# johannah/drqv2

Hardware: AMD Instinct MI355X
Metric: agent updates/sec (batch=256, 9x84x84 obs) (higher is better)
Workload: dtype f32; 1 GPU; cheetah_run batch_size=256/GPU (256 global) 9x84x84 u8 obs, A=6, feature_dim=50, hidden_dim=1024, fp32, use_tb=True; parallelism=dp1, global_batch=256

## Files before the change

drqv2_amd/_lib.py:

```python
import ctypes as C
import os

import torch

HERE = os.path.dirname(os.path.abspath(__file__))
LIB_PATH = os.path.join(HERE, "libdrqv2_hip.so")

c_float_p = C.c_void_p
c_u8_p = C.c_void_p
stream_t = C.c_void_p


class DrqStep(C.Structure):
    _fields_ = [
        ("B", C.c_int), ("global_B", C.c_int), ("C", C.c_int), ("A", C.c_int), ("F", C.c_int), ("H", C.c_int),
        ("obs", c_u8_p), ("next_obs", c_u8_p),
        ("action", c_float_p), ("reward", c_float_p), ("discount", c_float_p),
        ("shift_obs", c_float_p), ("shift_next", c_float_p),
        ("noise_critic", c_float_p), ("noise_actor", c_float_p),
        ("base_grid", c_float_p),
        ("params", c_float_p), ("grads", c_float_p), ("adam_m", c_float_p), ("adam_v", c_float_p),
        ("ws", c_float_p), ("ws_bytes", C.c_size_t),
        ("sums", c_float_p),
        ("lr", C.c_double), ("tau", C.c_double),
# ... 15 lines not shown

PROTOTYPES = {
    "drq_abi_version": (I, []),
    "drq_aug_fwd": (I, [P, P, P, P, I, I, I, I, I, P]),
    "drq_aug_fwd_f32": (I, [P, P, P, P, I, I, I, I, P]),
    "drq_conv1_aug_fwd": (I, [P, P, P, P, P, P, P, P, P, I, I, P]),
    "drq_conv1_aug_fwd_bf16": (I, [P, P, P, P, P, P, P, P, P, I, I, P]),
    "drq_conv1_aug_fwd_bf16_nhwc": (I, [P, P, P, P, P, P, P, P, P, I, I, P]),
    "drq_conv1_aug_fwd_indexed": (I, [P, P, P, P, P, P, P, P, P, P, P, I, I, P]),
    "drq_conv1_aug_fwd_frames": (I, [P, P, L, L, P, P, P, P, P, P, P, P, P, I, I, P]),
    "drq_conv1_aug_fwd_frames_bf16": (I, [P, P, L, L, P, P, P, P, P, P, P, P, P, I, I, P]),
    "drq_conv3x3_fwd": (I, [P, P, P, P, I, I, I, I, I, L, L, L, L, P]),
    "drq_conv3x3_dgrad": (I, [P, P, P, P, I, I, L, L, L, L, P]),
    "drq_conv3x3_fwd_wino": (I, [P, P, P, P, I, I, I, L, L, L, L, P]),
    "drq_conv3x3_dgrad_wino": (I, [P, P, P, P, I, I, L, L, L, L, P]),
    "drq_conv3x3_wgrad_wino": (I, [P, P, P, P, I, I, L, L, L, L, P, SZ, P]),
    "drq_conv3x3_wgrad": (I, [P, P, P, P, I, I, I, I, L, L, L, L, P, SZ, P]),
    "drq_conv3x3_wgrad_ws_bytes": (SZ, []),
    "drq_conv3x3_fwd_bf16": (I, [P, P, P, P, I, I, I, L, L, L, L, P]),
    "drq_conv3x3_dgrad_bf16": (I, [P, P, P, P, I, I, L, L, L, L, P]),
    "drq_conv3x3_wgrad_bf16": (I, [P, P, P, P, I, I, L, L, L, L, P, SZ, P]),
    "drq_conv3x3_fwd_bf16_nhwc": (I, [P, P, P, P, I, I, I, I, I, P]),
    "drq_conv3x3_dgrad_bf16_nhwc": (I, [P, P, P, P, I, I, I, I, L, L, L, L, P]),
    "drq_conv3x3_wgrad_bf16_nhwc": (I, [P, P, P, P, I, I, I, L, L, L, L, P, SZ, P]),
    "drq_gemm_f32": (I, [P, L, I, P, L, I, P, L, I, I, I, I, L, L, L, P, L, I, P, I, L, I, I, I, P, SZ, P]),
    "drq_gemm_batched_f32": (I, [I, P, L, I, P, L, I, P, L, I, I, I, P, I, P, I, P, I, I, I, P, SZ, P]),
    "drq_gemm_batched_bf16": (I, [I, P, L, I, P, L, I, P, L, I, I, I, P, I, P, I, P, I, I, P, SZ, P]),
    "drq_gemm_batched_partial": (I, [I, P, L, I, P, L, I, P, L, I, I, I, P, P, SZ, C.POINTER(I), P]),
    "drq_mlp_fwd": (I, [I, P, L, P, L, P, L, I, I, I, P, I, P, P, C.POINTER(I), P]),
    "drq_mlp_dgrad": (I, [I, P, L, P, L, P, L, I, I, I, P, I, P]),
# ... 49 lines not shown
    "drq_vec_video_record": (I, [P, P, I, P, I, P, I, I, I, L, P]),
    "drq_vec_export_rows": (I, [P, P, P, P, L, L, I, L, I, P, I, P, P, P, P, P]),
    "drq_vec_fill": (I, [P, P, P, P, P, L, L, I, L, L, I, P, P, P, P, P, P]),
    "drq_nstep_gather_frames": (I, [P, P, L, P, P, P, P, I, I, L, I, F, P, P, P, P, P, P]),
    "drq_relu_mask_pad": (I, [P, P, P, L, I, I, P]),
    "drq_conv1_dgrad": (I, [P, P, P, I, P]),
    "drq_aug_bwd_f32": (I, [P, P, P, P, I, I, I, I, P]),
    "drq_tanh_bwd": (I, [P, P, P, L, P]),
    "drq_dormant_scores": (I, [P, L, I, I, P, P]),
    "drq_dormant_count": (I, [P, I, F, P, P, P]),
    "drq_lerp_flat": (I, [P, P, L, F, P]),
    "drq_param_layout": (I, [I, I, I, I, C.POINTER(L), I]),
    "drq_step_ws_bytes": (SZ, [I, I, I, I, I]),
    "drq_step_ws_offset": (L, [I, I, I, I, I, I]),
    "drq_update_phase": (I, [C.POINTER(DrqStep), I]),
    "drq_update_phase_bc": (I, [C.POINTER(DrqStep), I, F]),
    "drq_update_phase_per": (I, [C.POINTER(DrqStep), I, P, P]),
    "drq_update_phase_frames": (I, [C.POINTER(DrqStep), I, P, L, L, P, P]),
    "drq_act_forward": (I, [C.POINTER(DrqStep), P, I, P]),
    "drq_act_ws_bytes": (SZ, [I, I, I, I, I]),
    "drq_act_batch": (I, [P, I, I, I, I, P, I, P, F, P, P, P, SZ, P]),
    "drq_publish_sums": (I, [P, P, C.c_uint, P]),
    "drq_rng_draws": (I, [C.c_uint64, C.c_uint64, I, I, I, P, P, P, P, P]),
}

WS_IDS = ["AUG", "ACT1", "ACT2", "ACT3", "FEAT", "Z_NEXT", "Z_OBS", "HA_T", "HA_C", "H_AN", "H_AO", "Q", "TQ",
          "DQ", "MU_O", "DY4", "DY3", "DY2", "DY1", "DZ_C", "DZ_A", "HA_C2", "P1", "P2", "C1", "C2"]

PHASE_ALL, PHASE_CRITIC, PHASE_ACTOR, PHASE_OPT = -1, 0, 1, 2
PHASE_ENCODE, PHASE_CRITIC_HEADS, PHASE_CONV_BACKWARD, PHASE_ACTOR_FORWARD, PHASE_ACTOR_BACKWARD = 3, 4, 5, 6, 7
PHASE_ENCODER_OPT, PHASE_ACTOR_OPT = 8, 9
PHASE_CRITIC_OPT, PHASE_ACTOR_LOSS, PHASE_POLYAK, PHASE_REDRAW = 10, 11, 12, 13

PARAM_LAYOUT_LEN = 59

NO_STREAM = frozenset({"drq_abi_version", "drq_conv3x3_wgrad_ws_bytes", "drq_param_layout", "drq_step_ws_bytes",
                       "drq_step_ws_offset", "drq_update_phase", "drq_update_phase_bc", "drq_update_phase_per",
                       "drq_update_phase_frames", "drq_act_forward", "drq_act_ws_bytes"})

_lib = None


class DrqError(RuntimeError):
    pass


def load():
    global _lib
    if _lib is not None:
        return _lib
    if not os.path.exists(LIB_PATH):
        raise DrqError(f"{LIB_PATH} is missing: build it with `python -m drqv2_amd.build` "
# ... 58 lines not shown
```

drqv2_amd/csrc/conv_plan.h:

```cpp
#pragma once
#include <cstddef>

constexpr int kEncH[5] = {84, 41, 39, 37, 35};
constexpr int kConvOk = 0, kConvEarg = -1, kConvEws = -2;

struct ConvView {
  long bs, cs, rs, off;
  static constexpr ConvView contiguous(int h) { return {32L * h * h, (long)h * h, h, 0}; }
  static constexpr ConvView padded(int h) { return {32L * (h + 4) * (h + 4), (long)(h + 4) * (h + 4), h + 4, 2L * (h + 4) + 2}; }
};
inline bool conv_bytes_ok(size_t nb, size_t frame, size_t elem_bytes = 4) { return nb * frame * elem_bytes < (1ull << 31); }
inline unsigned conv_bytes(size_t nb, size_t frame, size_t elem_bytes = 4) { return (unsigned)(nb * frame * elem_bytes); }
inline bool view_ok(int nb, const ConvView& v) { return v.off >= 0 && v.bs > 0 && conv_bytes_ok(nb, v.bs); }

constexpr int conv_part(bool small) { return (small ? 3 : 9) * 1024 + 64; }

constexpr int kConvBlk = 2, kConvTpw = 1;
constexpr int kConv1Bands = 5, kConv1MaxU = 64;
constexpr int conv_bf_wgs(int lay) { return (lay & 1) ? 3 : 2; }
constexpr int conv_bf_npart(int lay, int hin) { return conv_bf_wgs(lay) == 3 && hin >= 43 ? 4 : 3; }
constexpr bool conv_hin32_ok(int hin) { return hin == 41 || hin == 39 || hin == 37; }

struct ConvPlan {
  int rc = kConvOk;
// ... 17 lines not shown
  const int hout = (hin - 3) / stride + 1;
  const long ntiles = ((long)nb * hout * hout + 31) / 32;
  p.grid = conv_grid((ntiles + 8 * kConvTpw - 1) / (8 * kConvTpw), (long)kConvBlk * cus);
  return p;
}

inline ConvPlan plan_wgrad_direct(int cus, int nb, int cin, int hin, int stride, size_t part_bytes) {
  if (!(cin == 9 && hin == 84 && stride == 2) && !(cin == 32 && stride == 1 && conv_hin32_ok(hin))) return conv_refuse(kConvEarg);
  ConvPlan p;
  p.small = cin * 3 <= 32;
  const int hout = (hin - 3) / stride + 1;
  p.grid = p.records[0] = conv_grid(((long)nb * hout + 3) / 4, (p.small ? 2L : 1L) * cus);
  return conv_ws(p, p.grid, part_bytes);
}

inline ConvPlan plan_wino(int cus, int nb, int hin) {
  ConvPlan p;
  const int th = (hin - 1) / 2;
  const long nunit = ((long)nb * th * th + 15) / 16;
  p.grid = conv_grid((nunit + 3) / 4, 2L * cus);
  return p;
}

inline long conv_ww_steps(int nb, int hin) { return ((long)nb * ((hin - 1) / 2) * ((hin - 1) / 2) + 3) / 4; }

inline ConvPlan plan_ww(int cus, int nb, int hin, const ConvView& dy, size_t part_bytes) {
  const int hout = hin - 2;
  if (dy.rs < hout + 1 || dy.cs < (long)(hout + 1) * dy.rs) return conv_refuse(kConvEarg);
  ConvPlan p;
  p.grid = p.records[0] = conv_grid((conv_ww_steps(nb, hin) + 3) / 4, cus);
  return conv_ws(p, cus, part_bytes);
}

inline ConvPlan plan_ww3(int cus, int nb, size_t part_bytes) {
  long steps[3], tot = 0;
  for (int l = 0; l < 3; ++l) tot += steps[l] = conv_ww_steps(nb, kEncH[l + 1]);
// ... 53 lines not shown
```

drqv2_amd/csrc/conv_wino.hip:

```cpp
#include "common.h"
#include "internal.h"
#include "wino_u.h"
#include <type_traits>

namespace {

struct WinoArgs {
  const float* x;
  const float* w;
  const float* pre;
  const float* bias;
  const float* mask;
  float* y;
  int y_bs, y_cs, y_rs, y_off;
  unsigned x_bytes, y_bytes, mask_bytes;
  int nb;
  int relu;
  int wmode;
  int stagger;
};

typedef unsigned u32x4w __attribute__((ext_vector_type(4)));
typedef unsigned u32x2w __attribute__((ext_vector_type(2)));
typedef float f32x2w __attribute__((ext_vector_type(2)));
// ... 70 lines not shown
    for (int i = 0; i < 4; ++i) {
      const u32x4w v = __builtin_amdgcn_raw_buffer_load_b128(xrs, voff, c * (4 * PLANE) + i * (HIN * 4), 0);
      const unsigned e0 = v[0], e1 = v[1], e2 = v[2], e3 = v[3];
      d[i * 4 + 0] = __uint_as_float(e0);
      d[i * 4 + 1] = __uint_as_float(e1);
      d[i * 4 + 2] = __uint_as_float(e2);
      d[i * 4 + 3] = __uint_as_float(e3);
    }
  };

  auto load_A = [&](f32x2w (&A)[8], int c, int g) {
#pragma unroll
    for (int p = 0; p < 8; ++p) A[p] = Ul[((8 * g + p) * 8 + c) * 64];
  };

  const int hg = (int)gridDim.x >> 1;
  const int bh = (int)blockIdx.x >= hg ? 1 : 0, bl = (int)blockIdx.x - bh * hg;
  const int lb = ((int)gridDim.x & 15) ? (int)blockIdx.x : bh * hg + (bl & 7) * (hg >> 3) + (bl >> 3);
  const int gw = lb * 4 + wid;
  const int q = nunit / nwave, r = nunit - q * nwave;
  const int nf = 2 * r > nwave ? 2 * r - nwave : 0;
  const int nfull = q + (gw < nf ? 1 : 0);
  const int hk = gw - nf;
  const bool has_half = hk >= 0 && hk < 2 * (r - nf);
  const int half_unit = q * nwave + nf + (hk >> 1), half_h = hk & 1;
  auto item_unit = [&](int i) { return i < nfull ? gw + i * nwave : half_unit; };
  const int nitem = nfull + (has_half ? 1 : 0);

  float d[16];
  f32x2w A0[8], A1[8];
  int voff = 0;
  if (nitem > 0) {
    voff = patch_voff(item_unit(0));
    load_patch(d, voff, 0);
    load_A(A0, 0, 0);
  }
  auto body = [&](auto hsel_tag, int unit, int next_unit) {
    constexpr int HSEL = decltype(hsel_tag)::value;
    const int nvoff = patch_voff(next_unit);
    const int t0 = unit * 16 + tl;
// ... 125 lines not shown
    else body(std::integral_constant<int, 1>{}, half_unit, half_unit);
  }
}

template <int HIN>
int launch_wino(const WinoArgs& a, const ConvPlan& p, hipStream_t st) {
  const dim3 g((unsigned)p.grid), t(256);
  if (a.mask && a.relu) hipLaunchKernelGGL((conv3x3_wino_kernel<HIN, true, true>), g, t, 0, st, a);
  else if (a.mask) hipLaunchKernelGGL((conv3x3_wino_kernel<HIN, true, false>), g, t, 0, st, a);
  else if (a.relu) hipLaunchKernelGGL((conv3x3_wino_kernel<HIN, false, true>), g, t, 0, st, a);
  else hipLaunchKernelGGL((conv3x3_wino_kernel<HIN, false, false>), g, t, 0, st, a);
  return drq_launched();
}

int wino_any(bool dgrad, const float* x, const float* w, const float* u_image, const float* bias, const float* mask,
             float* y, int nb, int hin, int relu, const ConvView& yv, hipStream_t st) {
  if (!x || !w || !y || nb <= 0) return DRQ_EARG;
  const size_t frame = 32 * (size_t)hin * hin, mframe = 32 * ((size_t)hin - 2) * ((size_t)hin - 2);
  if (!conv_bytes_ok(nb, frame) || !view_ok(nb, yv)) return DRQ_EARG;
  const WinoArgs a{x, w, u_image, bias, mask, y, (int)yv.bs, (int)yv.cs, (int)yv.rs, (int)yv.off, conv_bytes(nb, frame),
                   conv_bytes(nb, yv.bs), dgrad ? conv_bytes(nb, mframe) : 0u, nb, relu, dgrad, kStagger};
  const ConvPlan p = plan_wino(drq_num_cus(), nb, hin);
  auto go = [&](auto h) { return launch_wino<decltype(h)::value>(a, p, st); };
  return dgrad ? drq_dispatch<39, 41, 43>(hin, go) : drq_dispatch<41, 39, 37>(hin, go);
}

}

int drq_conv3x3_fwd_wino_pre(const float* x, const float* w, const float* u_image, const float* bias, float* y, int nb,
                             int hin, int relu, ConvView yv, hipStream_t st) {
  return wino_any(false, x, w, u_image, bias, nullptr, y, nb, hin, relu, yv, st);
}

int drq_conv3x3_dgrad_wino_pre(const float* dy_pad, const float* w, const float* u_image, const float* mask, float* dx,
                               int nb, int hout, ConvView dxv, hipStream_t st) {
  return wino_any(true, dy_pad, w, u_image, nullptr, mask, dx, nb, hout + 4, 0, dxv, st);
}

DRQ_API int drq_conv3x3_fwd_wino(const float* x, const float* w, const float* bias, float* y, int nb, int hin, int relu,
                                 long y_bs, long y_cs, long y_rs, long y_off, hipStream_t st) {
  return drq_conv3x3_fwd_wino_pre(x, w, nullptr, bias, y, nb, hin, relu, {y_bs, y_cs, y_rs, y_off}, st);
}

DRQ_API int drq_conv3x3_dgrad_wino(const float* dy_pad, const float* w, const float* mask, float* dx, int nb, int hout,
                                   long dx_bs, long dx_cs, long dx_rs, long dx_off, hipStream_t st) {
  return drq_conv3x3_dgrad_wino_pre(dy_pad, w, nullptr, mask, dx, nb, hout, {dx_bs, dx_cs, dx_rs, dx_off}, st);
}
```

drqv2_amd/csrc/internal.h:

```cpp
#pragma once
#include "common.h"
#include "conv_plan.h"
#include "gemm_plan.h"

int drq_ln_tanh_fwd_multi_part(int n, const float* const* z, int ldz, const float* const* gamma,
                               const float* const* beta, float* const* out, const int* ldo, float* const* xhat,
                               float* const* rstd, int rows, int F, const float* const* tail, const int* tail_ld,
                               int tail_n, const float* part, const float* const* bias, int splitk, hipStream_t st);
int drq_ln_tanh_bwd_part(const float* dh0, int ld0, const float* dh1, int ld1, const float* h, int ldh,
                         const float* xhat, const float* rstd, const float* gamma, float* dz, float* dln,
                         float* dgamma, float* dbeta, int rows, int F, const float* part, int splitk, int nprob,
                         int ldp, hipStream_t st);
int drq_ln_param_grad(const float* dln, const float* xhat, float* dgamma, float* dbeta, int rows, int F,
                      hipStream_t st);

int drq_actor_loss_ex(const float* q1, const float* q2, const float* a, long lda, const float* a_beh, long ldb,
                      const float* mu, float std, float alpha, float* dq1, float* dq2, float* sums, int B, int A,
                      float inv_global_B, float* sums_host, unsigned seq, hipStream_t st);

int drq_qout_bwd_td(const float* tq1, const float* tq2, const float* q1, const float* q2, const float* reward,
                    const float* discount, const float* is_weight, float inv_global_B, float* sums, float* td_abs,
                    const float* const* h, const float* const* w, float* const* dh, float* const* dw, float* const* db,
                    int B, int H, hipStream_t st);
int drq_qout_bwd_actor(const float* q1, const float* q2, const float* act, long lda, const float* a_beh, long ldb,
// ... 61 lines not shown
                 const int* rows, const int* nheads, const float* const* w, const float* const* b, float* const* y, int F,
                 int H, int splitk, long slab, hipStream_t st);
int drq_polout_l1_fwd(const float* p2, const float* w3, const float* b3, float* p3, int rows, int srow0, int H, int A,
                      int F, float std, float clip, int use_clip, const float* noise_hi, float* mu_hi, float* ha_hi,
                      long lda_hi, const float* noise_lo, float* mu_lo, float* ha_lo, long lda_lo, int nheads,
                      const float* const* w, const float* const* b, float* const* y, hipStream_t st);

static_assert(kConvOk == DRQ_OK && kConvEarg == DRQ_EARG && kConvEws == DRQ_EWS, "ConvPlan::rc is the entry's result");
int drq_conv1_aug_fwd_any(int bf_mma, const uint8_t* obs, const float* shift, const uint8_t* obs1, const float* shift1,
                          const float* base_grid, const float* w, const float* bias, float* xaug, float* y, int n,
                          int n_store, hipStream_t st, const float* const* wino_w, float* wino_u, const long* fidx0,
                          const long* fidx1, const uint8_t* ring_first, long ring_R, long ring_N);
int drq_conv3x3_fwd_wino_pre(const float* x, const float* w, const float* u_image, const float* bias, float* y, int nb,
                             int hin, int relu, ConvView yv, hipStream_t st);
int drq_conv3x3_dgrad_wino_pre(const float* dy_pad, const float* w, const float* u_image, const float* mask, float* dx,
                               int nb, int hout, ConvView dxv, hipStream_t st);
int drq_conv3x3_fwd_bf16_lay(const void* x, const float* w, const float* bias, void* y, int nb, int hin, int relu,
                             ConvView yv, int lay, hipStream_t st);
int drq_conv3x3_dgrad_bf16_lay(const void* dy_pad, const float* w, const void* mask, void* dx, int nb, int hout,
                               ConvView dxv, int lay, hipStream_t st);
int drq_conv3x3_wgrad_partial_bf16_lay(const void* x, const void* dy, int nb, int hin, ConvView dyv, float* part,
                                       size_t part_bytes, int* nblocks, int lay, hipStream_t st);
int drq_conv3x3_wgrad_partial(const float* x, const float* dy, int nb, int cin, int hin, int stride, ConvView dyv,
                              float* part, size_t part_bytes, int* nblocks, hipStream_t st);
int drq_conv3x3_wgrad_reduce_multi(int n, const float* const* part, const int* nblocks, const int* cin,
                                   float* const* dw, float* const* db, hipStream_t st);
int drq_conv3x3_wgrad_reduce_one(int rc, const float* part, int nblocks, int cin, float* dw, float* db, hipStream_t st);
int drq_conv3x3_wgrad_partial_wino(const float* x, const float* dy, int nb, int hin, ConvView dyv, float* part,
                                   size_t part_bytes, int* nblocks, hipStream_t st);
int drq_conv3x3_wgrad_partial_wino3(const float* const* x, const float* const* dy, int nb, const ConvView* dyv,
                                    float* const* part, size_t part_bytes, int* nblocks, hipStream_t st);
// ... 20 lines not shown
```

drqv2_amd/csrc/step.hip:

```cpp
#include "common.h"
#include "internal.h"
#include "../../include/drqv2_hip.h"

namespace {

constexpr long R = 32L * 35 * 35;
inline long al64(long x) { return (x + 63) & ~63L; }
inline long al512(long x) { return (x + 511) & ~511L; }

struct HeadOff {
  long trunk_w, trunk_b, ln_g, ln_b;
  long w[2][3], b[2][3];
};
enum { SEG_ENC, SEG_CRITIC, SEG_ACTOR, SEG_TARGET };
struct ParamLayout {
  long enc_w[4], enc_b[4];
  HeadOff critic, actor, target;
  long seg[8];
  long total;
  long flat[50];
  int nflat;
  long seg_beg(int net) const { return seg[2 * net]; }
  long seg_len(int net) const { return seg[2 * net + 1] - seg[2 * net]; }
};
// ... 127 lines not shown
  w.total = off;
  return w;
}

#define CK(expr)                \
  do {                          \
    const int rc__ = (expr);    \
    if (rc__ != 0) return rc__; \
  } while (0)

struct Ctx {
  const DrqStep* s;
  ParamLayout P;
  WsLayout W;
  hipStream_t st;
  bool fuse_actor_loss = false;
  float bc_alpha = 0.f;
  bool bc() const { return bc_alpha > 0.f; }
  const float* a_beh() const { return bc() ? ws(W_HA_C) + s->F : nullptr; }
  float bc_scale() const { return 2.0f / ((float)s->global_B * (float)s->A); }
  const float* is_weight = nullptr;
  float* td_abs = nullptr;
  bool per() const { return is_weight != nullptr; }
  const uint8_t* ring_first = nullptr;
  long ring_R = 0, ring_N = 0;
  bool qout_loss_fits_lds() const { return ((size_t)s->B + 5 * 1024 + 16) * 4 <= 60 * 1024; }
  bool actor_loss_fused() const { return fuse_actor_loss && qout_loss_fits_lds(); }
  bool fuse_rows() const {
    return !(s->flags & DRQ_STEP_NO_ROW_FUSION) && !s->bf16 && s->A <= 32 && s->F + s->A <= 64 && s->F % 2 == 0 &&
           s->A % 2 == 0 && s->H % 256 == 0;
// ... 284 lines not shown
                          c.ws(W_RSTD_C), c.p(cr.ln_g), c.ws(W_DZ_C), c.ws(W_DLN), ride ? nullptr : c.g(cr.ln_g),
                          ride ? nullptr : c.g(cr.ln_b), B, F, sk_dha > 1 ? c.gemm_ws() : nullptr, sk_dha, 2, FA, st));
  {
    const float *dz[1] = {c.ws(W_DZ_C)}, *w[1] = {c.p(cr.trunk_w)}, *mk[1] = {feat_obs};
    float* dy4[1] = {c.ws(W_DY4)};
    CK(c.trunk_wgrad(c.ws(W_DZ_C), feat_obs, c.g(cr.trunk_w), c.g(cr.trunk_b), ride, c.ws(W_DLN), c.ws(W_XHAT_C),
                     c.g(cr.ln_g), c.g(cr.ln_b)));
    GemmCall dfeat = c.gemm(1, dz, F, 1, w, R, 0, dy4, 0, B, (int)R, F);
    dfeat.bf16 = false; dfeat.aux_p = mk; dfeat.ldaux = (int)R; dfeat.scatter_hw = 35;
    CK(drq_gemm_batched_any(dfeat));
  }

  return 0;
}

int phase_conv_backward(const Ctx& c) {
  const DrqStep* s = c.s;
  const ParamLayout& P = c.P;
  const int B = s->B, C = s->C;
  hipStream_t st = c.st;
  const int dyid[4] = {W_DY1, W_DY2, W_DY3, W_DY4};
  const int actid[4] = {W_AUG, W_ACT1, W_ACT2, W_ACT3};
  float* cws = c.ws(W_CONV_WS);
  const size_t quarter = drq_conv3x3_wgrad_ws_bytes() / 4;
  const float *parts[4], *xs[4], *dys[4];
  int nblk[4], cins[4];
  float *dws[4], *dbs[4], *ps[4];
  ConvView dyv[4];
  const bool wino = !c.bf16();
  for (int l = 0; l < 4; ++l) {
    xs[l] = c.ws(actid[l]); dys[l] = c.ws(dyid[l]); dyv[l] = ConvView::padded(kEncH[l + 1]);
    parts[l] = ps[l] = cws + (size_t)l * (quarter / sizeof(float));
    cins[l] = l == 0 ? C : 32; dws[l] = c.g(P.enc_w[l]); dbs[l] = c.g(P.enc_b[l]);
  }
  for (int l = 3; l >= 1; --l) {
    if (!wino)
      CK(drq_conv3x3_wgrad_partial_bf16_lay(xs[l], dys[l], B, kEncH[l], dyv[l], ps[l], quarter, &nblk[l],
                                            (c.acts16() ? 1 : 0) | (c.grads16() && l < 3 ? 2 : 0), st));
    if (l == 2) CK(c.stamp(2));
    if (!wino)
      CK(drq_conv3x3_dgrad_bf16_lay(dys[l], c.p(P.enc_w[l]), xs[l], c.ws(dyid[l - 1]), B, kEncH[l + 1], dyv[l - 1],
                                    (c.acts16() ? 4 : 0) | (c.grads16() && l < 3 ? 1 : 0) | (c.grads16() && l > 1 ? 2 : 0),
                                    st));
    else
      CK(drq_conv3x3_dgrad_wino_pre(dys[l], c.p(P.enc_w[l]), c.ws(W_WINO_U) + (2L * (l - 1) + 1) * 16384, xs[l],
                                    c.ws(dyid[l - 1]), B, kEncH[l + 1], dyv[l - 1], st));
    if (l == 2) CK(c.stamp(3));
  }
  if (wino) {
    CK(c.stamp(4));
    if (plan_ww3(drq_num_cus(), B, quarter).merged)
      CK(drq_conv3x3_wgrad_partial_wino3(xs + 1, dys + 1, B, dyv + 1, ps + 1, quarter, nblk + 1, st));
    else
      for (int l = 1; l < 4; ++l)
        CK(drq_conv3x3_wgrad_partial_wino(xs[l], dys[l], B, kEncH[l], dyv[l], ps[l], quarter, &nblk[l], st));
    CK(c.stamp(5));
  }
  CK(drq_conv3x3_wgrad_partial(xs[0], dys[0], B, C, kEncH[0], 2, dyv[0], ps[0], quarter, &nblk[0], st));
  CK(drq_conv3x3_wgrad_reduce_multi(4, parts, nblk, cins, dws, dbs, st));
  return 0;
}
// ... 125 lines not shown
                          c.ws(W_DZ_A), c.ws(W_DLN), ride ? nullptr : c.g(ac.ln_g), ride ? nullptr : c.g(ac.ln_b), B, F,
                          sk_dh > 1 ? c.gemm_ws() : nullptr, sk_dh, 1, F, st));
  CK(c.trunk_wgrad(c.ws(W_DZ_A), feat_obs, c.g(ac.trunk_w), c.g(ac.trunk_b), ride, c.ws(W_DLN), c.ws(W_XHAT_A),
                   c.g(ac.ln_g), c.g(ac.ln_b)));
  return 0;
}

int phase_both_opt(const Ctx& c) {
  const DrqStep* s = c.s;
  const ParamLayout& P = c.P;
  const long e = P.seg_beg(SEG_ENC), a = P.seg_beg(SEG_ACTOR);
  return drq_adam_flat2(c.p(e), c.g(e), s->adam_m + e, s->adam_v + e, P.seg_len(SEG_ENC), s->step_enc, c.p(a), c.g(a),
                        s->adam_m + a, s->adam_v + a, P.seg_len(SEG_ACTOR), s->step_actor, s->lr, s->gscale, c.st);
}

bool runs(int phase, int part) {
  switch (phase) {
    case DRQ_PHASE_ALL: return (part >= DRQ_PHASE_ENCODE && part <= DRQ_PHASE_ACTOR_BACKWARD) || part == DRQ_PHASE_OPT;
    case DRQ_PHASE_CRITIC: return part >= DRQ_PHASE_ENCODE && part <= DRQ_PHASE_CONV_BACKWARD;
    case DRQ_PHASE_ACTOR: return part == DRQ_PHASE_ACTOR_FORWARD || part == DRQ_PHASE_ACTOR_BACKWARD;
    default: return phase == part;
  }
}

int check_step(const DrqStep* s) {
  if (!s) return DRQ_EARG;
  if (s->B <= 0 || s->global_B < s->B || s->C <= 0 || s->C > 32 || s->A <= 0 || s->F <= 0 || s->F > 256 || s->H <= 0)
    return DRQ_EARG;
  if (s->C != 9) return DRQ_EARG;
  if (!s->params || !s->ws) return DRQ_EARG;
// ... 16 lines not shown
  return n;
}

DRQ_API size_t drq_step_ws_bytes(int B, int C, int A, int F, int H) {
  if (B <= 0 || C <= 0 || A <= 0 || F <= 0 || H <= 0) return 0;
  return (size_t)ws_layout(B, C, A, F, H).total * sizeof(float);
}

DRQ_API long drq_step_ws_offset(int B, int C, int A, int F, int H, int id) {
  if (id < 0 || id >= DRQ_WS_NBUF_PUBLIC) return -1;
  return ws_layout(B, C, A, F, H).off[id];
}

namespace {
int update_phase(const DrqStep* s, int phase, float bc_alpha, const float* is_weight = nullptr, float* td_abs = nullptr,
                 const uint8_t* ring_first = nullptr, long ring_R = 0, long ring_N = 0) {
  CK(check_step(s));
  if (!s->obs || !s->next_obs || !s->action || !s->reward || !s->discount || !s->shift_obs || !s->shift_next ||
      !s->noise_critic || !s->noise_actor || !s->base_grid || !s->grads || !s->adam_m || !s->adam_v || !s->sums)
    return DRQ_EARG;
  Ctx c{s, param_layout(s->C, s->A, s->F, s->H), ws_layout(s->B, s->C, s->A, s->F, s->H), (hipStream_t)s->stream};
  if (phase < DRQ_PHASE_ALL || phase > DRQ_PHASE_REDRAW) return DRQ_EARG;
  c.fuse_actor_loss = phase == DRQ_PHASE_ALL || phase == DRQ_PHASE_ACTOR;
  c.bc_alpha = bc_alpha;
  c.is_weight = is_weight;
  c.td_abs = td_abs;
  c.ring_first = ring_first;
  c.ring_R = ring_R;
  c.ring_N = ring_N;
  if (runs(phase, DRQ_PHASE_ENCODE)) CK(phase_encode(c));
  if (runs(phase, DRQ_PHASE_CRITIC_HEADS)) {
    CK(c.stamp(6));
    CK(phase_critic_heads(c));
    CK(c.stamp(7));
  }
  if (runs(phase, DRQ_PHASE_CONV_BACKWARD)) CK(phase_conv_backward(c));
  if (runs(phase, DRQ_PHASE_ACTOR_FORWARD)) CK(phase_actor_forward(c));
  if (runs(phase, DRQ_PHASE_ACTOR_BACKWARD)) {
    CK(phase_actor_backward(c));
    CK(c.stamp(9));
  }
  if (runs(phase, DRQ_PHASE_OPT)) CK(phase_both_opt(c));
  if (runs(phase, DRQ_PHASE_ENCODER_OPT)) CK(c.adam_segment(SEG_ENC, s->step_enc));
  if (runs(phase, DRQ_PHASE_ACTOR_OPT)) CK(c.adam_segment(SEG_ACTOR, s->step_actor));
  if (runs(phase, DRQ_PHASE_CRITIC_OPT)) CK(c.adam_segment(SEG_CRITIC, s->step_critic));
  if (runs(phase, DRQ_PHASE_ACTOR_LOSS)) CK(phase_actor_forward(c, false));
  if (runs(phase, DRQ_PHASE_POLYAK))
    CK(drq_ema_flat(c.p(c.P.seg_beg(SEG_CRITIC)), c.p(c.P.seg_beg(SEG_TARGET)), c.P.seg_len(SEG_CRITIC), s->tau, c.st));
  if (runs(phase, DRQ_PHASE_REDRAW)) {
    const int F = s->F, A = s->A, FA = F + A;
    CK(drq_trunc_normal_sample(c.ws(W_P3), s->noise_actor, s->std, s->clip, 1, c.ws(W_MU_O), c.ws(W_HA_C2) + F, FA, s->B,
                               A, c.st));
  }
  return 0;
}
}

DRQ_API int drq_update_phase(const DrqStep* s, int phase) { return update_phase(s, phase, 0.f); }

DRQ_API int drq_update_phase_bc(const DrqStep* s, int phase, float bc_alpha) {
  if (!(bc_alpha > 0.f) || bc_alpha > 3.0e38f || (s && s->global_B != s->B)) return DRQ_EARG;
  return update_phase(s, phase, bc_alpha);
}

DRQ_API int drq_update_phase_per(const DrqStep* s, int phase, const float* is_weight, float* td_abs) {
  if (!is_weight || !td_abs || (s && s->global_B != s->B)) return DRQ_EARG;
  return update_phase(s, phase, 0.f, is_weight, td_abs);
}

DRQ_API int drq_update_phase_frames(const DrqStep* s, int phase, const uint8_t* first, long R, long N,
                                    const float* is_weight, float* td_abs) {
  if (!first || R <= 0 || N <= 0 || (is_weight != nullptr) != (td_abs != nullptr)) return DRQ_EARG;
  if (s && (!s->obs_index || !s->next_obs_index || s->obs != s->next_obs || s->global_B != s->B)) return DRQ_EARG;
// ... 56 lines not shown
```

drqv2_amd/engine.py:

```python
import ctypes

import torch

from . import _lib
from ._lib import DrqStep, check, launch, ptr

NETS = ("enc", "critic", "actor", "target")


class FlatAdam(torch.optim.Optimizer):

    def __init__(self, params, lr, seg_p, seg_g, seg_m, seg_v, grad_views=None, flush=None):
        params = list(params)
        super().__init__(params, dict(lr=lr, betas=(0.9, 0.999), eps=1e-8, weight_decay=0, amsgrad=False))
        self._p, self._g, self._m, self._v = seg_p, seg_g, seg_m, seg_v
        self._views = list(zip(params, grad_views)) if grad_views is not None else []
        self._flush = flush
        self.t = 0

    @property
    def lr(self):
        return self.param_groups[0]["lr"]

    def begin_step(self):
# ... 255 lines not shown
        self._last_seq = None
        self._enqueued = []
        self.pg = None
        self._pending = None
        self._pending_enc = None
        self.global_metrics = False
        self._timing_array = None
        self._timing_n = 0
        self.step_flags = 0
        self.metrics_spin = 256
        self.metrics_wait_est = None
        self.profile_exchange = False
        self.exchange_wait_us = {}
        self._wait_events = []
        self._side = None
        self._side_busy = False
        self.bf16 = False
        self.store_aug_next = False
        self.world = 1
        self.rank = 0
        self.exchange = None
        self.fused_rng = True
        self._rng_ok = None
        self._rng_bufs = None
        self._td_bufs = None
        self.last_td_abs = None

    def _adopt(self, name, mod):
        offs = self.layout[name]
        plist = list(mod.parameters())
# ... 302 lines not shown
                                f"buffer with 32-bit byte offsets, which holds up to {self.MAX_BATCH} rows "
                                "(2B x 32 x 41 x 41 floats < 2 GiB): split the batch over more GPUs")
        B_global = B * self.world if B_global is None else B_global
        per = self._loss_weights(loss_weights, B) if loss_weights is not None else None
        steps = (self.critic_opt.begin_step(), self.encoder_opt.begin_step(), self.actor_opt.begin_step())
        d = self.make_desc(B, B_global, std, clip, tau, steps)
        keep = (obs, action, reward, discount, next_obs, shift_obs, shift_next, noise_critic, noise_actor, obs_index,
                next_obs_index, per, ring)
        d.obs, d.next_obs = ptr(obs), ptr(next_obs)
        d.obs_index, d.next_obs_index = ptr(obs_index), ptr(next_obs_index)
        d.action, d.reward, d.discount = ptr(action), ptr(reward), ptr(discount)
        d.shift_obs, d.shift_next = ptr(shift_obs), ptr(shift_next)
        d.noise_critic, d.noise_actor = ptr(noise_critic), ptr(noise_actor)
        if self.pg is None:
            self._throttle(steps[2] & 0xFFFFFFFF)
            self._phase(d, _lib.PHASE_ALL, per, ring)
            self.last_td_abs = per[1] if per is not None else None
            self._last_seq = steps[2] & 0xFFFFFFFF
        else:
            (c0, c1), (e0, e1), (a0, a1) = grad_buckets_overlap(self.layout)
            mirror = self.sums_host is not None
            seq = steps[2] & 0xFFFFFFFF
            if mirror:
                self._throttle(seq)
            if self._side_busy:
                torch.cuda.current_stream(self.device).wait_stream(self._side)
                self._side_busy = False
            self.flush_encoder()
            self._phase(d, _lib.PHASE_ENCODE)
            self.flush()
            self._phase(d, _lib.PHASE_CRITIC_HEADS)
# ... 287 lines not shown
```

include/drqv2_hip.h:

```cpp
#ifndef DRQV2_HIP_H
#define DRQV2_HIP_H
#include <stddef.h>
#include <stdint.h>

#ifdef __cplusplus
extern "C" {
#endif

typedef void* drq_stream_t;

#define DRQ_OK 0
#define DRQ_EARG (-1)
#define DRQ_EWS (-2)

int drq_abi_version(void);

int drq_aug_fwd(const uint8_t* obs, const float* shift_xy, const float* base_grid, float* out, int n, int c,
                int hw, int pad, int fuse_norm, drq_stream_t stream);
int drq_aug_fwd_f32(const float* x, const float* shift_xy, const float* base_grid, float* out, int n, int c,
                    int hw, int pad, drq_stream_t stream);

int drq_conv1_aug_fwd(const uint8_t* obs, const float* shift, const uint8_t* obs1, const float* shift1,
                      const float* base_grid, const float* w, const float* bias, float* xaug, float* y, int n,
                      int n_store, drq_stream_t stream);
// ... 11 lines not shown
int drq_conv1_aug_fwd_bf16(const uint8_t* obs, const float* shift, const uint8_t* obs1, const float* shift1,
                           const float* base_grid, const float* w, const float* bias, float* xaug, float* y, int n,
                           int n_store, drq_stream_t stream);
int drq_conv1_aug_fwd_bf16_nhwc(const uint8_t* obs, const float* shift, const uint8_t* obs1, const float* shift1,
                                const float* base_grid, const float* w, const float* bias, float* xaug, void* y_nhwc,
                                int n, int n_store, drq_stream_t stream);

int drq_conv3x3_fwd(const float* x, const float* w, const float* bias, float* y, int nb, int cin, int hin,
                    int stride, int relu, long y_bs, long y_cs, long y_rs, long y_off, drq_stream_t stream);
int drq_conv3x3_dgrad(const float* dy_pad, const float* w, const float* mask, float* dx, int nb, int hout,
                      long dx_bs, long dx_cs, long dx_rs, long dx_off, drq_stream_t stream);
int drq_conv3x3_fwd_wino(const float* x, const float* w, const float* bias, float* y, int nb, int hin, int relu,
                         long y_bs, long y_cs, long y_rs, long y_off, drq_stream_t stream);
int drq_conv3x3_dgrad_wino(const float* dy_pad, const float* w, const float* mask, float* dx, int nb, int hout,
                           long dx_bs, long dx_cs, long dx_rs, long dx_off, drq_stream_t stream);
int drq_conv3x3_wgrad_wino(const float* x, const float* dy, float* dw, float* db, int nb, int hin, long dy_bs,
                           long dy_cs, long dy_rs, long dy_off, float* ws, size_t ws_bytes, drq_stream_t stream);
int drq_conv3x3_wgrad(const float* x, const float* dy, float* dw, float* db, int nb, int cin, int hin,
                      int stride, long dy_bs, long dy_cs, long dy_rs, long dy_off, float* ws, size_t ws_bytes,
                      drq_stream_t stream);
size_t drq_conv3x3_wgrad_ws_bytes(void);

int drq_conv3x3_fwd_bf16(const float* x, const float* w, const float* bias, float* y, int nb, int hin, int relu,
                         long y_bs, long y_cs, long y_rs, long y_off, drq_stream_t stream);
int drq_conv3x3_dgrad_bf16(const float* dy_pad, const float* w, const float* mask, float* dx, int nb, int hout,
                           long dx_bs, long dx_cs, long dx_rs, long dx_off, drq_stream_t stream);
int drq_conv3x3_wgrad_bf16(const float* x, const float* dy, float* dw, float* db, int nb, int hin, long dy_bs,
                           long dy_cs, long dy_rs, long dy_off, float* ws, size_t ws_bytes, drq_stream_t stream);
int drq_conv3x3_fwd_bf16_nhwc(const void* x, const float* w, const float* bias, void* y, int nb, int hin, int relu,
                              int x_nhwc, int y_nhwc, drq_stream_t stream);
// ... 222 lines not shown
  float gscale;
  drq_stream_t stream;
  float* sums_host;
  int store_aug_next;
  int bf16;
  void* const* timing_events;
  int timing_n;
  const int64_t* obs_index;
  const int64_t* next_obs_index;
  int flags;
} DrqStep;
#define DRQ_STEP_NO_ROW_FUSION 1
#define DRQ_STEP_NO_GEMM3 2
#define DRQ_STEP_BF16_FP32_ACTS 4
#define DRQ_STEP_BF16_FP32_GRADS 8

int drq_param_layout(int C, int A, int F, int H, long* out, int cap);
#define DRQ_PARAM_LAYOUT_LEN 59

size_t drq_step_ws_bytes(int B, int C, int A, int F, int H);
long drq_step_ws_offset(int B, int C, int A, int F, int H, int buffer_id);
enum {
  DRQ_WS_AUG = 0, DRQ_WS_ACT1, DRQ_WS_ACT2, DRQ_WS_ACT3, DRQ_WS_FEAT, DRQ_WS_Z_NEXT, DRQ_WS_Z_OBS,
  DRQ_WS_HA_T, DRQ_WS_HA_C, DRQ_WS_H_AN, DRQ_WS_H_AO, DRQ_WS_Q, DRQ_WS_TQ, DRQ_WS_DQ, DRQ_WS_MU_O,
  DRQ_WS_DY4, DRQ_WS_DY3, DRQ_WS_DY2, DRQ_WS_DY1, DRQ_WS_DZ_C, DRQ_WS_DZ_A, DRQ_WS_HA_C2,
  DRQ_WS_P1, DRQ_WS_P2,
  DRQ_WS_C1, DRQ_WS_C2,
  DRQ_WS_NBUF_PUBLIC
};

enum {
  DRQ_PHASE_ALL = -1, DRQ_PHASE_CRITIC = 0, DRQ_PHASE_ACTOR = 1, DRQ_PHASE_OPT = 2,
  DRQ_PHASE_ENCODE = 3, DRQ_PHASE_CRITIC_HEADS = 4, DRQ_PHASE_CONV_BACKWARD = 5, DRQ_PHASE_ACTOR_FORWARD = 6,
  DRQ_PHASE_ACTOR_BACKWARD = 7, DRQ_PHASE_ENCODER_OPT = 8, DRQ_PHASE_ACTOR_OPT = 9,
  DRQ_PHASE_CRITIC_OPT = 10, DRQ_PHASE_ACTOR_LOSS = 11, DRQ_PHASE_POLYAK = 12, DRQ_PHASE_REDRAW = 13
};
int drq_update_phase(const DrqStep* s, int phase);
int drq_update_phase_bc(const DrqStep* s, int phase, float bc_alpha);
int drq_update_phase_per(const DrqStep* s, int phase, const float* is_weight, float* td_abs);

int drq_update_phase_frames(const DrqStep* s, int phase, const uint8_t* first, long R, long N, const float* is_weight,
                            float* td_abs);

int drq_publish_sums(const float* sums, float* sums_host, unsigned seq, drq_stream_t stream);

int drq_act_forward(const DrqStep* s, const uint8_t* obs, int n, float* mu_out);

size_t drq_act_ws_bytes(int n_max, int C, int A, int F, int H);
int drq_act_batch(const float* params, int C, int A, int F, int H, const uint8_t* obs, int n, const float* noise,
                  float std, float* mu_out, float* action_out, void* ws, size_t ws_bytes, drq_stream_t stream);

#ifdef __cplusplus
// ... 4 lines not shown
```

Baseline: 974.2 updates/s.

## Overlap actor forward/backward with conv backward on a side stream

Runs the actor forward and backward phases on a side stream, forked and joined with events, concurrently with the encoder conv backward on the main stream. The Winograd dgrad grid is capped to a CU budget so the conv kernels leave compute units free for the actor kernels. The feature is enabled by default in the fp32 non-PER path. It adds event synchronisation overhead and a risk that the reduced conv grid slows the critical path if the overlap is small.

```diff
diff --git a/drqv2_amd/_lib.py b/drqv2_amd/_lib.py
--- a/drqv2_amd/_lib.py
+++ b/drqv2_amd/_lib.py
@@ -53,6 +53,7 @@
     "drq_conv3x3_dgrad": (I, [P, P, P, P, I, I, L, L, L, L, P]),
     "drq_conv3x3_fwd_wino": (I, [P, P, P, P, I, I, I, L, L, L, L, P]),
     "drq_conv3x3_dgrad_wino": (I, [P, P, P, P, I, I, L, L, L, L, P]),
+    "drq_conv3x3_dgrad_wino_budget": (I, [P, P, P, P, I, I, L, L, L, L, I, P]),
     "drq_conv3x3_wgrad_wino": (I, [P, P, P, P, I, I, L, L, L, L, P, SZ, P]),
     "drq_conv3x3_wgrad": (I, [P, P, P, P, I, I, I, I, L, L, L, L, P, SZ, P]),
     "drq_conv3x3_wgrad_ws_bytes": (SZ, []),
@@ -132,6 +133,7 @@
     "drq_step_ws_bytes": (SZ, [I, I, I, I, I]),
     "drq_step_ws_offset": (L, [I, I, I, I, I, I]),
     "drq_update_phase": (I, [C.POINTER(DrqStep), I]),
+    "drq_update_phase_overlap": (I, [C.POINTER(DrqStep), P, I]),
     "drq_update_phase_bc": (I, [C.POINTER(DrqStep), I, F]),
     "drq_update_phase_per": (I, [C.POINTER(DrqStep), I, P, P]),
     "drq_update_phase_frames": (I, [C.POINTER(DrqStep), I, P, L, L, P, P]),
@@ -150,10 +152,12 @@
 PHASE_ENCODER_OPT, PHASE_ACTOR_OPT = 8, 9
 PHASE_CRITIC_OPT, PHASE_ACTOR_LOSS, PHASE_POLYAK, PHASE_REDRAW = 10, 11, 12, 13
 
+STEP_OVERLAP_ACTOR = 16
+
 PARAM_LAYOUT_LEN = 59
 
 NO_STREAM = frozenset({"drq_abi_version", "drq_conv3x3_wgrad_ws_bytes", "drq_param_layout", "drq_step_ws_bytes",
-                       "drq_step_ws_offset", "drq_update_phase", "drq_update_phase_bc", "drq_update_phase_per",
+                       "drq_step_ws_offset", "drq_update_phase", "drq_update_phase_overlap", "drq_update_phase_bc", "drq_update_phase_per",
                        "drq_update_phase_frames", "drq_act_forward", "drq_act_ws_bytes"})
 
 _lib = None
diff --git a/drqv2_amd/csrc/conv_plan.h b/drqv2_amd/csrc/conv_plan.h
--- a/drqv2_amd/csrc/conv_plan.h
+++ b/drqv2_amd/csrc/conv_plan.h
@@ -55,12 +55,45 @@
   return conv_ws(p, p.grid, part_bytes);
 }
 
-inline ConvPlan plan_wino(int cus, int nb, int hin) {
+inline long wino_units(int nb, int hin) { return ((long)nb * ((hin - 1) / 2) * ((hin - 1) / 2) + 15) / 16; }
+inline ConvPlan plan_wino(int cus, int nb, int hin, int budget = 0) {
   ConvPlan p;
-  const int th = (hin - 1) / 2;
-  const long nunit = ((long)nb * th * th + 15) / 16;
-  p.grid = conv_grid((nunit + 3) / 4, 2L * cus);
+  long cap = 2L * cus;
+  if (budget > 0 && budget < cap) cap = budget < 16 ? 16 : budget & ~15;
+  p.grid = conv_grid((wino_units(nb, hin) + 3) / 4, cap);
   return p;
+}
+constexpr int kWinoOverlapBudget512 = 224;
+inline int wino_overlap_budget(int cus, int budget512 = kWinoOverlapBudget512) {
+  return (int)(2L * cus * budget512 / 512);
+}
+
+#ifdef __HIPCC__
+#define CONV_PLAN_HD __host__ __device__
+#else
+#define CONV_PLAN_HD
+#endif
+struct WinoDeal {
+  int gw, nwave;
+  int nfull;
+  bool has_half;
+  int half_unit, half_h;
+};
+CONV_PLAN_HD inline WinoDeal wino_deal(int grid, int block, int wid, int nunit) {
+  WinoDeal d;
+  const int hg = grid >> 1;
+  const int bh = block >= hg ? 1 : 0, bl = block - bh * hg;
+  const int lb = (grid & 15) ? block : bh * hg + (bl & 7) * (hg >> 3) + (bl >> 3);
+  d.gw = lb * 4 + wid;
+  d.nwave = grid * 4;
+  const int q = nunit / d.nwave, r = nunit - q * d.nwave;
+  const int nf = 2 * r > d.nwave ? 2 * r - d.nwave : 0;
+  d.nfull = q + (d.gw < nf ? 1 : 0);
+  const int hk = d.gw - nf;
+  d.has_half = hk >= 0 && hk < 2 * (r - nf);
+  d.half_unit = q * d.nwave + nf + (hk >> 1);
+  d.half_h = hk & 1;
+  return d;
 }
 
 inline long conv_ww_steps(int nb, int hin) { return ((long)nb * ((hin - 1) / 2) * ((hin - 1) / 2) + 3) / 4; }
diff --git a/drqv2_amd/csrc/conv_wino.hip b/drqv2_amd/csrc/conv_wino.hip
--- a/drqv2_amd/csrc/conv_wino.hip
+++ b/drqv2_amd/csrc/conv_wino.hip
@@ -108,16 +108,11 @@
     for (int p = 0; p < 8; ++p) A[p] = Ul[((8 * g + p) * 8 + c) * 64];
   };
 
-  const int hg = (int)gridDim.x >> 1;
-  const int bh = (int)blockIdx.x >= hg ? 1 : 0, bl = (int)blockIdx.x - bh * hg;
-  const int lb = ((int)gridDim.x & 15) ? (int)blockIdx.x : bh * hg + (bl & 7) * (hg >> 3) + (bl >> 3);
-  const int gw = lb * 4 + wid;
-  const int q = nunit / nwave, r = nunit - q * nwave;
-  const int nf = 2 * r > nwave ? 2 * r - nwave : 0;
-  const int nfull = q + (gw < nf ? 1 : 0);
-  const int hk = gw - nf;
-  const bool has_half = hk >= 0 && hk < 2 * (r - nf);
-  const int half_unit = q * nwave + nf + (hk >> 1), half_h = hk & 1;
+  const WinoDeal deal = wino_deal((int)gridDim.x, (int)blockIdx.x, wid, nunit);
+  const int gw = deal.gw;
+  const int nfull = deal.nfull;
+  const bool has_half = deal.has_half;
+  const int half_unit = deal.half_unit, half_h = deal.half_h;
   auto item_unit = [&](int i) { return i < nfull ? gw + i * nwave : half_unit; };
   const int nitem = nfull + (has_half ? 1 : 0);
 
@@ -273,13 +268,13 @@
 }
 
 int wino_any(bool dgrad, const float* x, const float* w, const float* u_image, const float* bias, const float* mask,
-             float* y, int nb, int hin, int relu, const ConvView& yv, hipStream_t st) {
-  if (!x || !w || !y || nb <= 0) return DRQ_EARG;
+             float* y, int nb, int hin, int relu, const ConvView& yv, hipStream_t st, int budget = 0) {
+  if (!x || !w || !y || nb <= 0 || budget < 0) return DRQ_EARG;
   const size_t frame = 32 * (size_t)hin * hin, mframe = 32 * ((size_t)hin - 2) * ((size_t)hin - 2);
   if (!conv_bytes_ok(nb, frame) || !view_ok(nb, yv)) return DRQ_EARG;
   const WinoArgs a{x, w, u_image, bias, mask, y, (int)yv.bs, (int)yv.cs, (int)yv.rs, (int)yv.off, conv_bytes(nb, frame),
                    conv_bytes(nb, yv.bs), dgrad ? conv_bytes(nb, mframe) : 0u, nb, relu, dgrad, kStagger};
-  const ConvPlan p = plan_wino(drq_num_cus(), nb, hin);
+  const ConvPlan p = plan_wino(drq_num_cus(), nb, hin, budget);
   auto go = [&](auto h) { return launch_wino<decltype(h)::value>(a, p, st); };
   return dgrad ? drq_dispatch<39, 41, 43>(hin, go) : drq_dispatch<41, 39, 37>(hin, go);
 }
@@ -292,8 +287,8 @@
 }
 
 int drq_conv3x3_dgrad_wino_pre(const float* dy_pad, const float* w, const float* u_image, const float* mask, float* dx,
-                               int nb, int hout, ConvView dxv, hipStream_t st) {
-  return wino_any(true, dy_pad, w, u_image, nullptr, mask, dx, nb, hout + 4, 0, dxv, st);
+                               int nb, int hout, ConvView dxv, hipStream_t st, int budget) {
+  return wino_any(true, dy_pad, w, u_image, nullptr, mask, dx, nb, hout + 4, 0, dxv, st, budget);
 }
 
 DRQ_API int drq_conv3x3_fwd_wino(const float* x, const float* w, const float* bias, float* y, int nb, int hin, int relu,
@@ -305,3 +300,9 @@
                                    long dx_bs, long dx_cs, long dx_rs, long dx_off, hipStream_t st) {
   return drq_conv3x3_dgrad_wino_pre(dy_pad, w, nullptr, mask, dx, nb, hout, {dx_bs, dx_cs, dx_rs, dx_off}, st);
 }
+
+DRQ_API int drq_conv3x3_dgrad_wino_budget(const float* dy_pad, const float* w, const float* mask, float* dx, int nb,
+                                          int hout, long dx_bs, long dx_cs, long dx_rs, long dx_off, int budget,
+                                          hipStream_t st) {
+  return drq_conv3x3_dgrad_wino_pre(dy_pad, w, nullptr, mask, dx, nb, hout, {dx_bs, dx_cs, dx_rs, dx_off}, st, budget);
+}
diff --git a/drqv2_amd/csrc/internal.h b/drqv2_amd/csrc/internal.h
--- a/drqv2_amd/csrc/internal.h
+++ b/drqv2_amd/csrc/internal.h
@@ -99,7 +99,7 @@
 int drq_conv3x3_fwd_wino_pre(const float* x, const float* w, const float* u_image, const float* bias, float* y, int nb,
                              int hin, int relu, ConvView yv, hipStream_t st);
 int drq_conv3x3_dgrad_wino_pre(const float* dy_pad, const float* w, const float* u_image, const float* mask, float* dx,
-                               int nb, int hout, ConvView dxv, hipStream_t st);
+                               int nb, int hout, ConvView dxv, hipStream_t st, int budget = 0);
 int drq_conv3x3_fwd_bf16_lay(const void* x, const float* w, const float* bias, void* y, int nb, int hin, int relu,
                              ConvView yv, int lay, hipStream_t st);
 int drq_conv3x3_dgrad_bf16_lay(const void* dy_pad, const float* w, const void* mask, void* dx, int nb, int hout,
diff --git a/drqv2_amd/csrc/step.hip b/drqv2_amd/csrc/step.hip
--- a/drqv2_amd/csrc/step.hip
+++ b/drqv2_amd/csrc/step.hip
@@ -1,6 +1,7 @@
 #include "common.h"
 #include "internal.h"
 #include "../../include/drqv2_hip.h"
+#include <mutex>
 
 namespace {
 
@@ -165,6 +166,7 @@
   ParamLayout P;
   WsLayout W;
   hipStream_t st;
+  hipStream_t side_st = nullptr;
   bool fuse_actor_loss = false;
   float bc_alpha = 0.f;
   bool bc() const { return bc_alpha > 0.f; }
@@ -479,7 +481,7 @@
   return 0;
 }
 
-int phase_conv_backward(const Ctx& c) {
+int phase_conv_backward(const Ctx& c, int igrad_budget = 0) {
   const DrqStep* s = c.s;
   const ParamLayout& P = c.P;
   const int B = s->B, C = s->C;
@@ -509,7 +511,7 @@
                                     st));
     else
       CK(drq_conv3x3_dgrad_wino_pre(dys[l], c.p(P.enc_w[l]), c.ws(W_WINO_U) + (2L * (l - 1) + 1) * 16384, xs[l],
-                                    c.ws(dyid[l - 1]), B, kEncH[l + 1], dyv[l - 1], st));
+                                    c.ws(dyid[l - 1]), B, kEncH[l + 1], dyv[l - 1], st, igrad_budget));
     if (l == 2) CK(c.stamp(3));
   }
   if (wino) {
@@ -665,6 +667,53 @@
                         s->adam_m + a, s->adam_v + a, P.seg_len(SEG_ACTOR), s->step_actor, s->lr, s->gscale, c.st);
 }
 
+struct ForkJoin {
+  hipEvent_t fork = nullptr, join = nullptr;
+};
+std::mutex g_fork_join_lock;
+int fork_join_events(ForkJoin** out) {
+  static ForkJoin table[64];
+  int dev = 0;
+  if (hipGetDevice(&dev) != hipSuccess || dev < 0 || dev >= 64) return DRQ_EARG;
+  ForkJoin& e = table[dev];
+  const unsigned fl = hipEventDisableTiming | hipEventDisableSystemFence;
+  if (!e.fork && hipEventCreateWithFlags(&e.fork, fl) != hipSuccess) { e.fork = nullptr; return DRQ_EARG; }
+  if (!e.join && hipEventCreateWithFlags(&e.join, fl) != hipSuccess) { e.join = nullptr; return DRQ_EARG; }
+  *out = &e;
+  return 0;
+}
+int order_after(hipStream_t from, hipStream_t to, bool join) {
+  std::lock_guard<std::mutex> hold(g_fork_join_lock);
+  ForkJoin* e = nullptr;
+  CK(fork_join_events(&e));
+  const hipEvent_t ev = join ? e->join : e->fork;
+  if (hipEventRecord(ev, from) != hipSuccess || hipStreamWaitEvent(to, ev, 0) != hipSuccess) return DRQ_EARG;
+  return 0;
+}
+
+bool overlap_actor(const Ctx& c, int phase) {
+  const DrqStep* s = c.s;
+  return phase == DRQ_PHASE_ALL && (s->flags & DRQ_STEP_OVERLAP_ACTOR) && c.side_st && c.side_st != c.st && !s->bf16 && !c.bc() && !c.per() && !c.ring_first && s->global_B == s->B &&
+         !(s->timing_events && s->timing_n > 0);
+}
+int overlap_budget(const DrqStep* s) {
+  const int n32 = (s->flags >> 8) & 63;
+  return n32 ? wino_overlap_budget(drq_num_cus(), n32 > 32 ? 512 : n32 * 16) : wino_overlap_budget(drq_num_cus());
+}
+
+int phases_backward_overlapped(const Ctx& c) {
+  const hipStream_t side_st = c.side_st;
+  CK(order_after(c.st, side_st, false));
+  Ctx side = c;
+  side.st = side_st;
+  side.side_st = nullptr;
+  const int rc_main = phase_conv_backward(c, overlap_budget(c.s));
+  int rc_side = phase_actor_forward(side);
+  if (rc_side == 0) rc_side = phase_actor_backward(side);
+  const int rc_join = order_after(side_st, c.st, true);
+  return rc_main ? rc_main : rc_side ? rc_side : rc_join;
+}
+
 bool runs(int phase, int part) {
   switch (phase) {
     case DRQ_PHASE_ALL: return (part >= DRQ_PHASE_ENCODE && part <= DRQ_PHASE_ACTOR_BACKWARD) || part == DRQ_PHASE_OPT;
@@ -711,7 +760,7 @@
 
 namespace {
 int update_phase(const DrqStep* s, int phase, float bc_alpha, const float* is_weight = nullptr, float* td_abs = nullptr,
-                 const uint8_t* ring_first = nullptr, long ring_R = 0, long ring_N = 0) {
+                 const uint8_t* ring_first = nullptr, long ring_R = 0, long ring_N = 0, hipStream_t side_st = nullptr) {
   CK(check_step(s));
   if (!s->obs || !s->next_obs || !s->action || !s->reward || !s->discount || !s->shift_obs || !s->shift_next ||
       !s->noise_critic || !s->noise_actor || !s->base_grid || !s->grads || !s->adam_m || !s->adam_v || !s->sums)
@@ -725,17 +774,22 @@
   c.ring_first = ring_first;
   c.ring_R = ring_R;
   c.ring_N = ring_N;
+  c.side_st = side_st;
   if (runs(phase, DRQ_PHASE_ENCODE)) CK(phase_encode(c));
   if (runs(phase, DRQ_PHASE_CRITIC_HEADS)) {
     CK(c.stamp(6));
     CK(phase_critic_heads(c));
     CK(c.stamp(7));
   }
-  if (runs(phase, DRQ_PHASE_CONV_BACKWARD)) CK(phase_conv_backward(c));
-  if (runs(phase, DRQ_PHASE_ACTOR_FORWARD)) CK(phase_actor_forward(c));
-  if (runs(phase, DRQ_PHASE_ACTOR_BACKWARD)) {
-    CK(phase_actor_backward(c));
-    CK(c.stamp(9));
+  if (overlap_actor(c, phase)) {
+    CK(phases_backward_overlapped(c));
+  } else {
+    if (runs(phase, DRQ_PHASE_CONV_BACKWARD)) CK(phase_conv_backward(c));
+    if (runs(phase, DRQ_PHASE_ACTOR_FORWARD)) CK(phase_actor_forward(c));
+    if (runs(phase, DRQ_PHASE_ACTOR_BACKWARD)) {
+      CK(phase_actor_backward(c));
+      CK(c.stamp(9));
+    }
   }
   if (runs(phase, DRQ_PHASE_OPT)) CK(phase_both_opt(c));
   if (runs(phase, DRQ_PHASE_ENCODER_OPT)) CK(c.adam_segment(SEG_ENC, s->step_enc));
@@ -754,6 +808,11 @@
 }
 
 DRQ_API int drq_update_phase(const DrqStep* s, int phase) { return update_phase(s, phase, 0.f); }
+
+DRQ_API int drq_update_phase_overlap(const DrqStep* s, drq_stream_t side_stream, int phase) {
+  if (!side_stream) return DRQ_EARG;
+  return update_phase(s, phase, 0.f, nullptr, nullptr, nullptr, 0, 0, (hipStream_t)side_stream);
+}
 
 DRQ_API int drq_update_phase_bc(const DrqStep* s, int phase, float bc_alpha) {
   if (!(bc_alpha > 0.f) || bc_alpha > 3.0e38f || (s && s->global_B != s->B)) return DRQ_EARG;
diff --git a/drqv2_amd/engine.py b/drqv2_amd/engine.py
--- a/drqv2_amd/engine.py
+++ b/drqv2_amd/engine.py
@@ -6,6 +6,7 @@
 from ._lib import DrqStep, check, launch, ptr
 
 NETS = ("enc", "critic", "actor", "target")
+OVERLAP_ACTOR_DEFAULT = True
 
 
 class FlatAdam(torch.optim.Optimizer):
@@ -293,6 +294,9 @@
         self.exchange_wait_us = {}
         self._wait_events = []
         self._side = None
+        self.overlap_actor = OVERLAP_ACTOR_DEFAULT
+        self.overlap_budget32 = 0
+        self._side_handle = None
         self._side_busy = False
         self.bf16 = False
         self.store_aug_next = False
@@ -625,7 +629,15 @@
         d.noise_critic, d.noise_actor = ptr(noise_critic), ptr(noise_actor)
         if self.pg is None:
             self._throttle(steps[2] & 0xFFFFFFFF)
-            self._phase(d, _lib.PHASE_ALL, per, ring)
+            if self.overlap_actor and per is None and ring is None and self.bc_alpha is None and not self.bf16:
+                if self._side_handle is None:
+                    self._side_handle = self._side_stream().cuda_stream
+                d.flags |= _lib.STEP_OVERLAP_ACTOR | ((int(self.overlap_budget32) & 63) << 8)
+                with torch.cuda.device(self.device):
+                    check(_lib.load().drq_update_phase_overlap(ctypes.byref(d), self._side_handle, _lib.PHASE_ALL),
+                          "drq_update_phase_overlap(-1)")
+            else:
+                self._phase(d, _lib.PHASE_ALL, per, ring)
             self.last_td_abs = per[1] if per is not None else None
             self._last_seq = steps[2] & 0xFFFFFFFF
         else:
diff --git a/include/drqv2_hip.h b/include/drqv2_hip.h
--- a/include/drqv2_hip.h
+++ b/include/drqv2_hip.h
@@ -49,6 +49,8 @@
                          long y_bs, long y_cs, long y_rs, long y_off, drq_stream_t stream);
 int drq_conv3x3_dgrad_wino(const float* dy_pad, const float* w, const float* mask, float* dx, int nb, int hout,
                            long dx_bs, long dx_cs, long dx_rs, long dx_off, drq_stream_t stream);
+int drq_conv3x3_dgrad_wino_budget(const float* dy_pad, const float* w, const float* mask, float* dx, int nb, int hout,
+                                  long dx_bs, long dx_cs, long dx_rs, long dx_off, int budget, drq_stream_t stream);
 int drq_conv3x3_wgrad_wino(const float* x, const float* dy, float* dw, float* db, int nb, int hin, long dy_bs,
                            long dy_cs, long dy_rs, long dy_off, float* ws, size_t ws_bytes, drq_stream_t stream);
 int drq_conv3x3_wgrad(const float* x, const float* dy, float* dw, float* db, int nb, int cin, int hin,
@@ -301,6 +303,8 @@
 #define DRQ_STEP_NO_GEMM3 2
 #define DRQ_STEP_BF16_FP32_ACTS 4
 #define DRQ_STEP_BF16_FP32_GRADS 8
+#define DRQ_STEP_OVERLAP_ACTOR 16
+#define DRQ_STEP_BUDGET(n) (((n) & 63) << 8)
 
 int drq_param_layout(int C, int A, int F, int H, long* out, int cap);
 #define DRQ_PARAM_LAYOUT_LEN 59
@@ -323,6 +327,7 @@
   DRQ_PHASE_CRITIC_OPT = 10, DRQ_PHASE_ACTOR_LOSS = 11, DRQ_PHASE_POLYAK = 12, DRQ_PHASE_REDRAW = 13
 };
 int drq_update_phase(const DrqStep* s, int phase);
+int drq_update_phase_overlap(const DrqStep* s, drq_stream_t side_stream, int phase);
 int drq_update_phase_bc(const DrqStep* s, int phase, float bc_alpha);
 int drq_update_phase_per(const DrqStep* s, int phase, const float* is_weight, float* td_abs);
 
```

Measured after the change: 1010 updates/s (median of 6 runs). 3.7% higher.
